# Pearbiossom-M/FlashAttention-from-Scratch-with-Triton

Hardware: AMD Instinct MI355X
Metric: achieved TFLOPS fwd and fwd+bwd (B=4,H=32,N=4096,D=64 causal); %MFMA peak (higher is better)
Workload: dtype bf16

## Files before the change

### flashattention-from-scratch-with-triton_amd/csrc/fa_fwd_v4.hip

```cpp
#include <stdlib.h>

#include <type_traits>

#include "fa_common.h"
#include "fa_kernels.h"

namespace fa {

template <int D_>
struct Fwd4Cfg {
  static constexpr int D = D_;
  static constexpr int BM = 256, NT = 256, NW = 4;
  static constexpr int BN = D == 64 ? 128 : 64;
  static constexpr int NBUF = D == 64 ? 3 : 4;
  static constexpr int NKB = BN / 32;
  static constexpr int ROWB = D * 2, CPR = D / 8, KS = D / 16, DB = D / 32;
  static constexpr int TILE_BYTES = BN * ROWB;
  static constexpr int V_BASE = NBUF * TILE_BYTES;
  static constexpr int FLAG_OFF = 2 * NBUF * TILE_BYTES;
  static constexpr int RB_BYTES = 32 * ROWB;
  static constexpr int QS_OFF = FLAG_OFF + 16;
  static constexpr int QS_BYTES = D == 64 ? 8 * RB_BYTES : 0;
  static constexpr int LDS_BYTES = QS_OFF + QS_BYTES;
  static constexpr int PIECES = TILE_BYTES / (NW * 1024);
  static constexpr int RPI = 1024 / ROWB;
#ifndef FA_FWD4_LSUM_MFMA
#define FA_FWD4_LSUM_MFMA 0
#endif
  static constexpr bool LSUM = FA_FWD4_LSUM_MFMA && D == 64;
  static constexpr int PVG = 2 * DB + (LSUM ? 2 : 0);
  static constexpr int NSS = 2 * KS, NPV = 2 * PVG, NSLOT = NSS + NPV;
  static constexpr int INFLIGHT = (NBUF - 3) * 2 * PIECES;
};

template <typename T> struct Fwd4Limit;
template <> struct Fwd4Limit<BF16> { static constexpr float value = 1.2676506e30f; };
template <> struct Fwd4Limit<FP16> { static constexpr float value = 32768.0f; };

#ifdef FA_STAMPS
#define FA4_STAMP(slot)                                                           \
  do {                                                                            \
    __builtin_amdgcn_sched_barrier(0);                                            \
    unsigned long long now_;                                                      \
    asm volatile("s_memtime %0\n\ts_waitcnt lgkmcnt(0)" : "=s"(now_)::"memory"); \
    __builtin_amdgcn_sched_barrier(0);                                            \
    seg[slot] += now_ - last_;                                                    \
    last_ = now_;                                                                 \
  } while (0)
#else
#define FA4_STAMP(slot) do {} while (0)
#endif

template <int D, typename T, bool CAUSAL>
__global__ __launch_bounds__(256, 1) void fa_fwd4_kernel(FwdParams p) {
#ifdef FA_STAMPS
  unsigned long long clk0_, rt0_;
  asm volatile("s_memtime %0\n\ts_memrealtime %1\n\ts_waitcnt lgkmcnt(0)" : "=s"(clk0_), "=s"(rt0_)::"memory");
  unsigned long long seg[12] = {0, 0, 0, 0, 0, 0, 0, 0, 0, 0, 0, 0};
  unsigned long long last_ = clk0_, ntile_ = 0, npass_ = 0;
#endif
  using C = Fwd4Cfg<D>;
  using vec8 = typename T::vec8;
  constexpr bool FOLD = T::kFoldScale;
  constexpr bool CHAIN_M = FOLD;
  extern __shared__ __attribute__((aligned(16))) char smem_raw[];
  FA_LDS char* smem = (FA_LDS char*)smem_raw;

  const int tid = threadIdx.x;
  const int lane = tid & 63;
  const int wave = __builtin_amdgcn_readfirstlane(tid >> 6);
  const int r = lane & 31, h = lane >> 5;

  const bool CONT = CAUSAL || (p.Sk % C::BN == 0 && p.Sk / C::BN >= C::NBUF - 1);
  constexpr bool STAGEQ = D == 64;
  const bool paired = CAUSAL && p.pair;
  const int nq = p.nq_tiles;
  const int per_bh = paired ? (nq + 1) / 2 : nq;
  const int n_items = per_bh * p.B * p.H;
  const int Sq = p.Sq, Sk = p.Sk;
  struct Work {
    int b, h, idx, npass;
  };
  auto decode = [&](int item) __attribute__((always_inline)) -> Work {
    const int w = xcd_remap(item, n_items);
    const int bh = p.div_per_bh.div(w), idx = w - bh * per_bh, b = p.div_h.div(bh);
    return Work{b, bh - b * p.H, idx, (paired && idx != nq - 1 - idx) ? 2 : 1};
  };
  auto tile_of = [&](const Work& wk, int pass) __attribute__((always_inline)) -> int {
    return paired ? (pass == 0 ? nq - 1 - wk.idx : wk.idx) : (CAUSAL ? nq - 1 - wk.idx : wk.idx);
  };

  const int q_rs = p.lq.rs, kv_rs = p.lk.rs, o_rs = p.lo.rs;
  auto rsrc_q = [&](const Work& wk, bool valid) __attribute__((always_inline)) {
    return make_rsrc((const char*)p.q + wk.b * p.lq.sb + wk.h * p.lq.sh, valid ? view_bytes(Sq, q_rs, C::ROWB) : 0u);
  };
  auto rsrc_k = [&](const Work& wk, bool valid) __attribute__((always_inline)) {
    return make_rsrc((const char*)p.k + wk.b * p.lk.sb + wk.h * p.lk.sh, valid ? view_bytes(Sk, kv_rs, C::ROWB) : 0u);
  };
  auto rsrc_v = [&](const Work& wk, bool valid) __attribute__((always_inline)) {
    return make_rsrc((const char*)p.v + wk.b * p.lv.sb + wk.h * p.lv.sh, valid ? view_bytes(Sk, kv_rs, C::ROWB) : 0u);
  };

  int dma_src[C::PIECES];
#pragma unroll
  for (int i = 0; i < C::PIECES; ++i) {
    const int row = (C::BN / C::NW) * wave + C::RPI * i + lane / C::CPR;
    dma_src[i] = row * kv_rs + swz_chunk<D>(row, lane % C::CPR) * 16 - 1024 * (i & 1);
  }
  int k_off[C::KS];
#pragma unroll
  for (int ks = 0; ks < C::KS; ++ks) k_off[ks] = lds_off<D>(r, 2 * ks + h);
  int v_off[2][C::DB];
#pragma unroll
  for (int e = 0; e < 2; ++e)
#pragma unroll
    for (int db = 0; db < C::DB; ++db) v_off[e][db] = tr_lane_off<D>(lane, 8 * e, db);
  const float c2 = p.scale * kLog2e;

  if (Sk % C::BN != 0) {
    lds_zero_fill(smem, C::FLAG_OFF, C::NT, tid);
    __syncthreads();
  }

  if (tid == 0) *(FA_LDS int*)(smem + C::FLAG_OFF) = 0;
  bool primed = false;
  int r0 = 0;

  int item = blockIdx.x, pass = 0;
  Work wk = decode(item);
  Work nwk_item = decode(min(item + (int)gridDim.x, n_items - 1));
  for (;;) {
    const int b_ = wk.b, h_ = wk.h;
    const __amdgpu_buffer_rsrc_t rk = rsrc_k(wk, true), rv = rsrc_v(wk, true);
    const __amdgpu_buffer_rsrc_t ro = make_rsrc((char*)p.o + b_ * p.lo.sb + h_ * p.lo.sh, view_bytes(Sq, o_rs, C::ROWB));
    const __amdgpu_buffer_rsrc_t rl = make_rsrc(p.lse + b_ * p.lse_sb + h_ * p.lse_sh, (unsigned)Sq * 4);
    const bool more_pass = pass + 1 < wk.npass, more_item = item + (int)gridDim.x < n_items;
    const bool has_next = CONT && (more_pass || more_item);
    const Work nwk = more_pass ? wk : nwk_item;
    const int nq0_wg = tile_of(nwk, more_pass ? pass + 1 : 0) * C::BM;

    FA4_STAMP(8);
    const int q0_wg = tile_of(wk, pass) * C::BM;
    const int qw = q0_wg + 32 * wave;
    auto qrow = [&](int rb) __attribute__((always_inline)) { return qw + 128 * rb; };

    const int kv_end = CAUSAL ? min(Sk, q0_wg + C::BM) : Sk;
    const int ntiles = (kv_end + C::BN - 1) / C::BN;
    const int nplain = CAUSAL ? min(Sk / C::BN, q0_wg / C::BN) : Sk / C::BN;

    auto dma_pair_of = [&](const __amdgpu_buffer_rsrc_t& rkx, const __amdgpu_buffer_rsrc_t& rvx, int t, int slot, int j) __attribute__((always_inline)) {
      constexpr int HALF = C::PIECES / 2;
      const int i = 2 * (j % HALF);
      const int dst = slot * C::TILE_BYTES + ((C::BN / C::NW) * wave + C::RPI * i) * C::ROWB;
      if (j < HALF) dma_pieces<2>(rkx, lds_addr_of(smem + dst), dma_src + i, t * C::BN * kv_rs);
      else dma_pieces<2>(rvx, lds_addr_of(smem + C::V_BASE + dst), dma_src + i, t * C::BN * kv_rs);
    };
    auto dma_pair = [&](int t, int slot, int j) __attribute__((always_inline)) { dma_pair_of(rk, rv, t, slot, j); };
    auto fetch_tile = [&](int t, int slot) __attribute__((always_inline)) {
#pragma unroll
      for (int j = 0; j < C::PIECES; ++j) dma_pair(t, slot, j);
    };
    auto stage_q_pair = [&](const __amdgpu_buffer_rsrc_t& rqx, int q0, int rb, int hf) __attribute__((always_inline)) {
      if constexpr (STAGEQ) {
        const int prow = lane >> 3;
        int voff[2];
#pragma unroll
        for (int i = 0; i < 2; ++i) {
          const int row = 8 * (2 * hf + i) + prow;
          voff[i] = (q0 + 128 * rb + 32 * wave + row) * q_rs + swz_chunk<D>(row, lane & 7) * 16 - 1024 * i;
        }
        dma_pieces<2>(rqx, lds_addr_of(smem + C::QS_OFF + (2 * wave + rb) * C::RB_BYTES + 2048 * hf), voff, 0);
      }
    };
    const bool was_primed = primed;
    if (!primed) {
      r0 = 0;
      if constexpr (STAGEQ) {
        const __amdgpu_buffer_rsrc_t rq = rsrc_q(wk, true);
#pragma unroll
        for (int g = 0; g < 4; ++g) stage_q_pair(rq, q0_wg, g >> 1, g & 1);
      }
#pragma unroll
      for (int t = 0; t < C::NBUF - 1; ++t) fetch_tile(t, t);
    }
    FA4_STAMP(9);
    u32x4 qf[2][C::KS];
    if constexpr (STAGEQ) {
      if (!was_primed) __builtin_amdgcn_s_waitcnt(0x0F70 | (((C::NBUF - 1) * 2 * C::PIECES) & 15) | ((((C::NBUF - 1) * 2 * C::PIECES) >> 4) << 14));
      asm volatile("" ::: "memory");
#pragma unroll
      for (int rb = 0; rb < 2; ++rb)
#pragma unroll
        for (int ks = 0; ks < C::KS; ++ks) {
          vec8 q = as_vec8<T>(lds_read16(smem + C::QS_OFF + (2 * wave + rb) * C::RB_BYTES + k_off[ks]));
          if constexpr (FOLD) q = scale_frag<T>(q, c2);
          qf[rb][ks] = __builtin_bit_cast(u32x4, q);
        }
    } else {
      const __amdgpu_buffer_rsrc_t rq = rsrc_q(wk, true);
#pragma unroll
      for (int rb = 0; rb < 2; ++rb)
#pragma unroll
        for (int ks = 0; ks < C::KS; ++ks) {
          vec8 q = as_vec8<T>(buf_load16(rq, (qrow(rb) + r) * q_rs + (2 * ks + h) * 16));
          if constexpr (FOLD) q = scale_frag<T>(q, c2);
          qf[rb][ks] = __builtin_bit_cast(u32x4, q);
        }
    }
    FA4_STAMP(10);
    int mask_base[2];
#pragma unroll
    for (int rb = 0; rb < 2; ++rb) mask_base[rb] = (CAUSAL ? min(qrow(rb) + r, Sk - 1) : Sk - 1) - 4 * h;

    auto commit = [&]() __attribute__((always_inline)) {
      asm volatile("" ::: "memory");
#ifdef FA_FWD4_COMMIT_LGKM0
      __builtin_amdgcn_s_waitcnt(0x0070 | (C::INFLIGHT & 15) | ((C::INFLIGHT >> 4) << 14));
#else
      __builtin_amdgcn_s_waitcnt(0x0F70 | (C::INFLIGHT & 15) | ((C::INFLIGHT >> 4) << 14));
#endif
      __builtin_amdgcn_s_barrier();
      asm volatile("" ::: "memory");
    };

    f32x16 S_[2][2];
    f32x16 negm[CHAIN_M ? 2 : 1];
    float mrow[2], nmc[2];
    float l[2];
    u32x4 pk[2][2][2];
#ifdef FA_FWD4_KR_FULL
    constexpr int KR = C::KS;
#else
    constexpr int KR = C::KS < 4 ? C::KS : 4;
#endif
    u32x4 KF[KR];
    vec8 VF[2 * C::DB];
    f32x16 oacc[2][C::DB];
    f32x16 lacc[C::LSUM ? 2 : 1];
    const unsigned one2 = std::is_same<T, BF16>::value ? 0x3F803F80u : 0x3C003C00u;
    const u32x4 ones = {one2, one2, one2, one2};
    int thr[2][2];

    auto block_valu = [&](int tau, f32x16 (&X)[2], u32x4 (&PK)[2][2], const int (&TH)[2], auto mask_tag, auto has0_tag) __attribute__((always_inline)) {
      constexpr bool MASK = decltype(mask_tag)::value, HAS0 = decltype(has0_tag)::value;
      auto first_q = [](int t) { return t <= 0 ? 0 : (32 * t + C::NSLOT - 1) / C::NSLOT; };
      auto work = [&](int t, bool exps) __attribute__((always_inline)) {
        if (t < 0 || t >= C::NSLOT) return;
#pragma unroll
        for (int u = 0; u < 2; ++u) {
          const int q = first_q(t) + u;
          if (q >= first_q(t + 1) || q >= 32) continue;
          const int rb = (q >> 3) & 1, e = (q & 7) + 8 * (q >> 4);
          if (rb == 0 && !HAS0) continue;
          if (exps) {
            float x = CHAIN_M ? X[rb][e] : (FOLD ? X[rb][e] + nmc[rb] : __builtin_fmaf(X[rb][e], c2, nmc[rb]));
            if constexpr (MASK) x = (e & 3) + 8 * (e >> 2) > TH[rb] ? -INFINITY : x;
            X[rb][e] = __builtin_amdgcn_exp2f(x);
          } else {
            if constexpr (!C::LSUM) l[rb] += X[rb][e];
            if (q & 1) {
              const int j = e >> 1;
              PK[rb][j >> 2][j & 3] = pack2<T>(X[rb][e - 1], X[rb][e]);
            }
          }
        }
      };
      work(tau - C::NSS, true);
      work(tau - 1 - C::NSS, false);
    };
    auto block_iter = [&](auto j_tag, auto set_tag, auto mode_tag, auto pst_tag, int kb0, const int (&kc)[C::KS], int kc_imm,
                          const int (&kn)[C::KS], int kn_delta, int kn_imm,
                          const int (&vc)[2][C::DB], int vc_imm, int vp0, int vp1, int vp_imm,
                          auto&& hook) __attribute__((always_inline)) {
      constexpr int J = decltype(j_tag)::value, SET = decltype(set_tag)::value, PSET = SET ^ 1;
      constexpr int MODE = decltype(mode_tag)::value, PST = decltype(pst_tag)::value;
      constexpr bool OWN0 = MODE != 3, PREV0 = PST != 2;
      using OwnMask = std::integral_constant<bool, MODE != 0>;
      using PrevMask = std::integral_constant<bool, PST != 0>;
      if constexpr (MODE != 0) {
        thr[SET][0] = mask_base[0] - kb0;
        thr[SET][1] = MODE == 2 ? (1 << 20) : mask_base[1] - kb0;
      }
#pragma unroll
      for (int s = 0; s < C::NSLOT; ++s) {
        hook(J, s);
        if (s < C::NSS) {
          const int ks = s >> 1, rb = s & 1;
          if (rb == 1 || OWN0) {
            if (ks == 0) {
              if constexpr (CHAIN_M) T::mfma_v_first(S_[SET][rb], KF[0], qf[rb][0], negm[CHAIN_M ? rb : 0]);
              else T::mfma_v_first0(S_[SET][rb], KF[0], qf[rb][0]);
            } else {
              T::mfma_v_acc(S_[SET][rb], KF[ks % KR], qf[rb][ks]);
            }
          }
        } else {
          const int n = s - C::NSS, e = n / C::PVG, m = n % C::PVG, rb = m & 1;
          if (rb == 1 || PREV0) {
            if (m < 2 * C::DB) oacc[rb][m >> 1] = T::mfma(VF[e * C::DB + (m >> 1)], as_vec8<T>(pk[PSET][rb][e]), oacc[rb][m >> 1]);
            else lacc[rb] = T::mfma(as_vec8<T>(ones), as_vec8<T>(pk[PSET][rb][e]), lacc[rb]);
          }
        }
        if (s >= 2 && s <= C::NSS && (s & 1) == 0) {
          const int ks = (s - 2) >> 1, nk = ks + KR;
          if (nk < C::KS) KF[ks % KR] = lds_read16(lds_at(kc[nk] + kc_imm));
          else KF[ks % KR] = lds_read16(lds_at(kn[nk - C::KS] + kn_delta + kn_imm));
        }
#pragma unroll
        for (int pp = 0; pp < 2 * C::DB; ++pp) {
          const int e = pp / C::DB, db = pp % C::DB, at = C::NSS + e * C::PVG + 2 * db + 2;
          if (at < C::NSLOT && s == at)
            VF[pp] = lds_read_tr_frag<T>(lds_at(vc[0][db] + vc_imm + 16 * e * C::ROWB), lds_at(vc[1][db] + vc_imm + 16 * e * C::ROWB));
          if (at >= C::NSLOT && s == 0)
            VF[pp] = lds_read_tr_frag<T>(lds_at(vp0 + vp_imm), lds_at(vp1 + vp_imm));
        }
        block_valu(C::NSLOT + s, S_[PSET], pk[PSET], thr[PSET], PrevMask{}, std::integral_constant<bool, PREV0>{});
        block_valu(s, S_[SET], pk[SET], thr[SET], OwnMask{}, std::integral_constant<bool, OWN0>{});
        if constexpr (CHAIN_M) {
          if (s == 1 && OWN0) keep_live(negm[0]);
          if (s == 2) keep_live(negm[CHAIN_M ? 1 : 0]);
        }
        __builtin_amdgcn_sched_barrier(0);
      }
    };
    auto drain = [&](auto set_tag, auto pst_tag, int rt_last) __attribute__((always_inline)) {
      constexpr int PSET = decltype(set_tag)::value ^ 1, PST = decltype(pst_tag)::value;
      constexpr bool PREV0 = PST != 2;
      if constexpr (!C::LSUM) {
        const int base = C::V_BASE + rt_last * C::TILE_BYTES + (C::NKB - 1) * 32 * C::ROWB + 16 * C::ROWB;
        VF[2 * C::DB - 1] = lds_read_tr_frag<T>(smem + v_off[0][C::DB - 1] + base, smem + v_off[1][C::DB - 1] + base);
      }
#pragma unroll
      for (int s = 0; s < C::NSLOT; ++s) {
        if (s >= C::NSS) {
          const int n = s - C::NSS, e = n / C::PVG, m = n % C::PVG, rb = m & 1;
          if (rb == 1 || PREV0) {
            if (m < 2 * C::DB) oacc[rb][m >> 1] = T::mfma(VF[e * C::DB + (m >> 1)], as_vec8<T>(pk[PSET][rb][e]), oacc[rb][m >> 1]);
            else lacc[rb] = T::mfma(as_vec8<T>(ones), as_vec8<T>(pk[PSET][rb][e]), lacc[rb]);
          }
        }
        block_valu(C::NSLOT + s, S_[PSET], pk[PSET], thr[PSET], std::integral_constant<bool, PST != 0>{}, std::integral_constant<bool, PREV0>{});
        __builtin_amdgcn_sched_barrier(0);
      }
    };

    auto tile_step = [&](int t, int rt, auto mode_tag, auto pst_tag, auto nx_tag) __attribute__((always_inline)) {
      constexpr int MODE = decltype(mode_tag)::value, NX = decltype(nx_tag)::value;
      const __amdgpu_buffer_rsrc_t nrk = rsrc_k(nwk, has_next && NX != 0), nrv = rsrc_v(nwk, has_next && NX != 0);
      const __amdgpu_buffer_rsrc_t nrq = rsrc_q(nwk, has_next && NX == 2);
      using OwnSt = std::integral_constant<int, MODE == 0 ? 0 : (MODE == 3 ? 2 : 1)>;
      const int rn = rt + 1 == C::NBUF ? 0 : rt + 1, rp = rt == 0 ? C::NBUF - 1 : rt - 1;
      const int lds0 = (int)lds_addr_of(smem);
      int kA[C::KS], vA[2][C::DB], vP[2];
      const int kdelta = (rn - rt) * C::TILE_BYTES;
#pragma unroll
      for (int ks = 0; ks < C::KS; ++ks) {
        kA[ks] = opaque(lds0 + k_off[ks] + rt * C::TILE_BYTES);
      }
#pragma unroll
      for (int e = 0; e < 2; ++e) {
#pragma unroll
        for (int db = 0; db < C::DB; ++db) vA[e][db] = opaque(lds0 + v_off[e][db] + C::V_BASE + rt * C::TILE_BYTES);
        vP[e] = opaque(lds0 + v_off[e][C::DB - 1] + C::V_BASE + (t == 0 ? rt * C::TILE_BYTES
                                                                  : rp * C::TILE_BYTES + (C::NKB - 1) * 32 * C::ROWB) + 16 * C::ROWB);
      }
      auto hook = [&](int J, int s) __attribute__((always_inline)) {
        if (J == C::NKB - 1) {
          if (s == 1) commit();
#pragma unroll
          for (int j = 0; j < C::PIECES; ++j)
            if (s == C::NSS + 1 + 2 * j) {
              if constexpr (NX != 0) dma_pair_of(nrk, nrv, t + C::NBUF - 1 - ntiles, rp, j);
              else dma_pair(t + C::NBUF - 1, rp, j);
            }
        }
        if constexpr (NX == 2 && STAGEQ) {
          if (J < 2 && s == C::NSS + 1) stage_q_pair(nrq, nq0_wg, J, 0);
          if (J < 2 && s == C::NSS + 5) stage_q_pair(nrq, nq0_wg, J, 1);
        }
      };
      auto go = [&](auto j_tag) __attribute__((always_inline)) {
        constexpr int J = decltype(j_tag)::value;
        constexpr int kPrevImm = (J - 1) * 32 * C::ROWB + 16 * C::ROWB;
        if constexpr (J == 0)
          block_iter(j_tag, std::integral_constant<int, 0>{}, mode_tag, pst_tag, t * C::BN, kA, 0, kA, 0, 32 * C::ROWB, vA, 0, vP[0], vP[1], 0, hook);
        else if constexpr (J + 1 < C::NKB)
          block_iter(j_tag, std::integral_constant<int, J & 1>{}, mode_tag, OwnSt{}, t * C::BN + 32 * J, kA, J * 32 * C::ROWB, kA, 0,
                     (J + 1) * 32 * C::ROWB, vA, J * 32 * C::ROWB, vA[0][C::DB - 1], vA[1][C::DB - 1], kPrevImm, hook);
        else
          block_iter(j_tag, std::integral_constant<int, J & 1>{}, mode_tag, OwnSt{}, t * C::BN + 32 * J, kA, J * 32 * C::ROWB, kA, kdelta, 0,
                     vA, J * 32 * C::ROWB, vA[0][C::DB - 1], vA[1][C::DB - 1], kPrevImm, hook);
      };
      go(std::integral_constant<int, 0>{});
      go(std::integral_constant<int, 1>{});
      if constexpr (C::NKB == 4) {
        go(std::integral_constant<int, 2>{});
        go(std::integral_constant<int, 3>{});
      }
    };

    auto scout_block = [&](const FA_LDS char* kblk, int kb0, float (&mx)[2]) __attribute__((always_inline)) {
#pragma unroll
      for (int rb = 0; rb < 2; ++rb) {
        f32x16 s;
        T::mfma_v_first0(s, lds_read16(kblk + k_off[0]), qf[rb][0]);
#pragma unroll
        for (int ks = 1; ks < C::KS; ++ks) T::mfma_v_acc(s, lds_read16(kblk + k_off[ks]), qf[rb][ks]);
        settle_mfma(s);
        const int th = opaque(mask_base[rb] - kb0);
        float mm = mx[rb];
#pragma unroll
        for (int i = 0; i < 16; ++i) mm = __builtin_fmaxf(mm, (i & 3) + 8 * (i >> 2) > th ? -INFINITY : s[i]);
        mx[rb] = mm;
      }
    };
    auto set_m = [&](const float (&mx)[2]) __attribute__((always_inline)) {
#pragma unroll
      for (int rb = 0; rb < 2; ++rb) {
        const float m = half_max(mx[rb]);
        mrow[rb] = m > -INFINITY ? m : 0.f;
        nmc[rb] = FOLD ? -mrow[rb] : -mrow[rb] * c2;
        if constexpr (CHAIN_M) {
#pragma unroll
          for (int i = 0; i < 16; ++i) negm[rb][i] = -mrow[rb];
        }
      }
    };

    for (int attempt = 0; attempt < 2; ++attempt) {
      if (attempt == 1) {
        r0 = 0;
#pragma unroll
        for (int t = 0; t < C::NBUF - 1; ++t) fetch_tile(t, t);
      }
      if (!was_primed || attempt == 1) {
        asm volatile("" ::: "memory");
        __builtin_amdgcn_s_waitcnt(0x0070 | (((C::NBUF - 2) * 2 * C::PIECES) & 15) | ((((C::NBUF - 2) * 2 * C::PIECES) >> 4) << 14));
        __builtin_amdgcn_s_barrier();
        asm volatile("" ::: "memory");
      }

      FA4_STAMP(0);
      float mx[2] = {-INFINITY, -INFINITY};
      if (attempt == 0) {
        scout_block(smem + r0 * C::TILE_BYTES, 0, mx);
        set_m(mx);
      } else {
        for (int t = 0; t < ntiles; ++t) {
          if (t > 0) {
            __syncthreads();
            fetch_tile(t, t % C::NBUF);
            __builtin_amdgcn_s_waitcnt(0x0070);
            __syncthreads();
          }
          for (int j = 0; j < C::NKB; ++j)
            scout_block(smem + (t % C::NBUF) * C::TILE_BYTES + j * 32 * C::ROWB, t * C::BN + 32 * j, mx);
        }
        set_m(mx);
        __builtin_amdgcn_s_waitcnt(0x0070);
        __syncthreads();
#pragma unroll
        for (int t = 0; t < C::NBUF - 1; ++t) fetch_tile(t, t);
        asm volatile("" ::: "memory");
        __builtin_amdgcn_s_waitcnt(0x0070 | (((C::NBUF - 2) * 2 * C::PIECES) & 15) | ((((C::NBUF - 2) * 2 * C::PIECES) >> 4) << 14));
        __builtin_amdgcn_s_barrier();
        asm volatile("" ::: "memory");
      }

      FA4_STAMP(1);
#pragma unroll
      for (int rb = 0; rb < 2; ++rb) {
        l[rb] = 0.f;
#pragma unroll
        for (int i = 0; i < 16; ++i) {
          const int q = (i >> 3) * 16 + rb * 8 + (i & 7);
          S_[1][rb][i] = C::NSS + q * C::NSLOT / 32 < C::NSLOT ? 0.f : -INFINITY;
        }
#pragma unroll
        for (int e = 0; e < 2; ++e) pk[1][rb][e] = u32x4{0u, 0u, 0u, 0u};
#pragma unroll
        for (int db = 0; db < C::DB; ++db)
#pragma unroll
          for (int i = 0; i < 16; ++i) oacc[rb][db][i] = 0.f;
        if constexpr (C::LSUM) {
#pragma unroll
          for (int i = 0; i < 16; ++i) lacc[rb][i] = 0.f;
        }
        thr[0][rb] = thr[1][rb] = 1 << 20;
      }
#pragma unroll
      for (int ks = 0; ks < KR; ++ks) KF[ks] = lds_read16(smem + r0 * C::TILE_BYTES + k_off[ks]);
#pragma unroll
      for (int pp = 0; pp < 2 * C::DB; ++pp) VF[pp] = as_vec8<T>(u32x4{0u, 0u, 0u, 0u});
      __builtin_amdgcn_sched_barrier(0);

      FA4_STAMP(2);
      int t = 0, rt = r0;
      using I0 = std::integral_constant<int, 0>;
      using I1 = std::integral_constant<int, 1>;
      using I2 = std::integral_constant<int, 2>;
      using I3 = std::integral_constant<int, 3>;
      const int nloop = (!CAUSAL && CONT) ? nplain - (C::NBUF - 1) : nplain;
      for (; t < nloop; ++t, rt = rt + 1 == C::NBUF ? 0 : rt + 1) tile_step(t, rt, I0{}, I0{}, I0{});
#ifdef FA_STAMPS
      FA4_STAMP(3);
      ntile_ += nplain;
      ++npass_;
#endif
      constexpr int RT = 256 / C::BN;
      auto nxt = [](int x) __attribute__((always_inline)) { return x + 1 == C::NBUF ? 0 : x + 1; };
      if constexpr (CAUSAL) {
        int rt_last;
        if constexpr (RT == 2) {
          tile_step(t, rt, I2{}, I1{}, I2{});
          tile_step(t + 1, rt_last = nxt(rt), I3{}, I1{}, I1{});
        } else {
          tile_step(t, rt, I2{}, I1{}, I0{});
          tile_step(t + 1, nxt(rt), I2{}, I1{}, I1{});
          tile_step(t + 2, nxt(nxt(rt)), I3{}, I1{}, I1{});
          tile_step(t + 3, rt_last = nxt(nxt(nxt(rt))), I3{}, I2{}, I1{});
        }
        static_assert(C::NBUF - 1 == (RT == 2 ? 2 : 3), "the masked tiles carry exactly the next pass's first NBUF - 1 tiles");
        FA4_STAMP(4);
        drain(I0{}, I2{}, rt_last);
        rt = rt_last;
      } else {
        if (CONT) {
          if constexpr (C::NBUF == 3) {
            tile_step(t, rt, I0{}, I0{}, I2{});
            tile_step(t + 1, nxt(rt), I0{}, I0{}, I1{});
            rt = nxt(nxt(rt));
          } else {
            tile_step(t, rt, I0{}, I0{}, I1{});
            tile_step(t + 1, nxt(rt), I0{}, I0{}, I1{});
            tile_step(t + 2, nxt(nxt(rt)), I0{}, I0{}, I1{});
            rt = nxt(nxt(nxt(rt)));
          }
          t += C::NBUF - 1;
        }
        for (; t < ntiles; ++t, rt = nxt(rt)) tile_step(t, rt, I1{}, I1{}, I0{});
        rt = rt == 0 ? C::NBUF - 1 : rt - 1;
        FA4_STAMP(4);
        drain(I0{}, I1{}, rt);
      }
      FA4_STAMP(5);

      float lt[2];
      bool bad = false;
#pragma unroll
      for (int rb = 0; rb < 2; ++rb) {
        lt[rb] = C::LSUM ? lacc[C::LSUM ? rb : 0][0] : half_sum(l[rb]);
        bad = bad || !(lt[rb] <= Fwd4Limit<T>::value);
      }
      FA_LDS int* flag = (FA_LDS int*)(smem + C::FLAG_OFF);
      if (attempt == 0 && __builtin_amdgcn_ballot_w64(bad) != 0 && lane == 0) *flag = 1;
      if (CONT) __builtin_amdgcn_s_waitcnt(0x0070 | (((C::NBUF - 2) * 2 * C::PIECES) & 15) | ((((C::NBUF - 2) * 2 * C::PIECES) >> 4) << 14));
      else __builtin_amdgcn_s_waitcnt(0x0070);
      __syncthreads();
      const int redo = __builtin_amdgcn_readfirstlane(*flag);
      FA4_STAMP(6);
      if (!redo) {
        FA_LDS char* stage = smem + (wave >> 1) * C::V_BASE + rt * C::TILE_BYTES + (wave & 1) * 32 * C::ROWB;
#pragma unroll
        for (int rb = 0; rb < 2; ++rb) {
          const float inv = lt[rb] > 0.f ? 1.0f / lt[rb] : 0.f;
          store_tile_rows<D, T>(oacc[rb], inv, stage, ro, qrow(rb) * o_rs, lane, o_rs);
          if (h == 0)
            buf_store_f32(rl, (qrow(rb) + r) * 4, mrow[rb] * (FOLD ? kLn2 : p.scale) + __builtin_logf(lt[rb]));
        }
        FA4_STAMP(7);
        primed = has_next;
        r0 = rt + 1 == C::NBUF ? 0 : rt + 1;
        break;
      }
      __builtin_amdgcn_s_waitcnt(0x0F70);
      __syncthreads();
      if (tid == 0) {
        *flag = 0;
#ifndef FA_STAMPS
        if (p.dbg) atomicAdd((unsigned*)p.dbg, 1u);
#endif
      }
    }
    if (more_pass) {
      ++pass;
    } else {
      item += gridDim.x;
      if (item >= n_items) break;
      wk = nwk_item;
      nwk_item = decode(min(item + (int)gridDim.x, n_items - 1));
      pass = 0;
    }
  }
#ifdef FA_STAMPS
  if (p.dbg && lane == 0) {
    unsigned long long* d = (unsigned long long*)p.dbg + ((size_t)blockIdx.x * 4 + wave) * 16;
    for (int i = 0; i < 12; ++i) d[i] = seg[i];
    d[12] = npass_;
    d[13] = ntile_;
    unsigned long long clk1_, rt1_;
    asm volatile("s_memtime %0\n\ts_memrealtime %1\n\ts_waitcnt lgkmcnt(0)" : "=s"(clk1_), "=s"(rt1_)::"memory");
    d[14] = clk1_ - clk0_;
    d[15] = rt1_ - rt0_;
  }
#endif
}

template <int D, typename T, bool CAUSAL>
static hipError_t launch4(const FwdParams& p, hipStream_t s) {
  using C = Fwd4Cfg<D>;
  int grid = (CAUSAL && p.pair ? (p.nq_tiles + 1) / 2 : p.nq_tiles) * p.B * p.H;
  if (CAUSAL || (p.Sk % C::BN == 0 && p.Sk / C::BN >= C::NBUF - 1)) {
    static std::atomic<int> cus{0};
    int n = cus.load(std::memory_order_relaxed);
    if (n == 0) {
      int dev = 0;
      if (hipGetDevice(&dev) != hipSuccess || hipDeviceGetAttribute(&n, hipDeviceAttributeMultiprocessorCount, dev) != hipSuccess || n < 8) n = 256;
      n -= n % 8;
      cus.store(n, std::memory_order_relaxed);
    }
    if (grid > n) grid = n;
  }
  auto kern = fa_fwd4_kernel<D, T, CAUSAL>;
  static std::atomic<unsigned long long> opted_in{0};
  if (hipError_t e = opt_in_lds((const void*)kern, C::LDS_BYTES, opted_in)) return e;
  hipLaunchKernelGGL(kern, dim3(grid), dim3(C::NT), C::LDS_BYTES, s, p);
  return hipGetLastError();
}

hipError_t launch_fwd_v4(FwdParams p, int D, int dtype, int causal, hipStream_t s) {
  p.nq_tiles = (p.Sq + 255) / 256;
  p.pair = causal != 0;
  p.div_per_bh = make_fastdiv(p.pair ? (p.nq_tiles + 1) / 2 : p.nq_tiles);
  p.div_h = make_fastdiv(p.H);
#define FA_GO(DD, TT) (causal ? launch4<DD, TT, true>(p, s) : launch4<DD, TT, false>(p, s))
  if (D == 64) return dtype == 1 ? FA_GO(64, BF16) : FA_GO(64, FP16);
  if (D == 128) return dtype == 1 ? FA_GO(128, BF16) : FA_GO(128, FP16);
#undef FA_GO
  return hipErrorInvalidValue;
}

}
```

Measured before the change: 888.7.

## Add per-wave diagonal walk for causal D=64 masked tiles with reversed Q row blocks

```diff
diff --git a/flashattention-from-scratch-with-triton_amd/csrc/fa_fwd_v4.hip b/flashattention-from-scratch-with-triton_amd/csrc/fa_fwd_v4.hip
--- a/flashattention-from-scratch-with-triton_amd/csrc/fa_fwd_v4.hip
+++ b/flashattention-from-scratch-with-triton_amd/csrc/fa_fwd_v4.hip
@@ -33,6 +33,9 @@
   static constexpr int INFLIGHT = (NBUF - 3) * 2 * PIECES;
 };
 
+constexpr int wait_vm(int n) { return 0x0F70 | (n & 15) | ((n >> 4) << 14); }
+constexpr int wait_vm_lgkm0(int n) { return 0x0070 | (n & 15) | ((n >> 4) << 14); }
+
 template <typename T> struct Fwd4Limit;
 template <> struct Fwd4Limit<BF16> { static constexpr float value = 1.2676506e30f; };
 template <> struct Fwd4Limit<FP16> { static constexpr float value = 32768.0f; };
@@ -116,6 +119,8 @@
 #pragma unroll
     for (int db = 0; db < C::DB; ++db) v_off[e][db] = tr_lane_off<D>(lane, 8 * e, db);
   const float c2 = p.scale * kLog2e;
+  const int qblk1 = D == 64 ? 128 + 32 * (3 - wave) : 128 + 32 * wave;
+  auto qblk = [&](int rb) __attribute__((always_inline)) { return D == 64 && rb == 1 ? qblk1 : 32 * wave + 128 * rb; };
 
   if (Sk % C::BN != 0) {
     lds_zero_fill(smem, C::FLAG_OFF, C::NT, tid);
@@ -142,7 +147,7 @@
     FA4_STAMP(8);
     const int q0_wg = tile_of(wk, pass) * C::BM;
     const int qw = q0_wg + 32 * wave;
-    auto qrow = [&](int rb) __attribute__((always_inline)) { return qw + 128 * rb; };
+    auto qrow = [&](int rb) __attribute__((always_inline)) { return D == 64 && rb == 1 ? q0_wg + qblk1 : qw + 128 * rb; };
 
     const int kv_end = CAUSAL ? min(Sk, q0_wg + C::BM) : Sk;
     const int ntiles = (kv_end + C::BN - 1) / C::BN;
@@ -167,7 +172,7 @@
 #pragma unroll
         for (int i = 0; i < 2; ++i) {
           const int row = 8 * (2 * hf + i) + prow;
-          voff[i] = (q0 + 128 * rb + 32 * wave + row) * q_rs + swz_chunk<D>(row, lane & 7) * 16 - 1024 * i;
+          voff[i] = (q0 + qblk(rb) + row) * q_rs + swz_chunk<D>(row, lane & 7) * 16 - 1024 * i;
         }
         dma_pieces<2>(rqx, lds_addr_of(smem + C::QS_OFF + (2 * wave + rb) * C::RB_BYTES + 2048 * hf), voff, 0);
       }
@@ -274,10 +279,10 @@
                           auto&& hook) __attribute__((always_inline)) {
       constexpr int J = decltype(j_tag)::value, SET = decltype(set_tag)::value, PSET = SET ^ 1;
       constexpr int MODE = decltype(mode_tag)::value, PST = decltype(pst_tag)::value;
-      constexpr bool OWN0 = MODE != 3, PREV0 = PST != 2;
-      using OwnMask = std::integral_constant<bool, MODE != 0>;
-      using PrevMask = std::integral_constant<bool, PST != 0>;
-      if constexpr (MODE != 0) {
+      constexpr bool OWN0 = MODE < 3, PREV0 = PST < 2;
+      using OwnMask = std::integral_constant<bool, MODE >= 1 && MODE <= 3>;
+      using PrevMask = std::integral_constant<bool, PST == 1 || PST == 2>;
+      if constexpr (OwnMask::value) {
         thr[SET][0] = mask_base[0] - kb0;
         thr[SET][1] = MODE == 2 ? (1 << 20) : mask_base[1] - kb0;
       }
@@ -323,11 +328,11 @@
         __builtin_amdgcn_sched_barrier(0);
       }
     };
-    auto drain = [&](auto set_tag, auto pst_tag, int rt_last) __attribute__((always_inline)) {
+    auto drain = [&](auto set_tag, auto pst_tag, int rt_last, int kb_last = C::NKB - 1) __attribute__((always_inline)) {
       constexpr int PSET = decltype(set_tag)::value ^ 1, PST = decltype(pst_tag)::value;
-      constexpr bool PREV0 = PST != 2;
+      constexpr bool PREV0 = PST < 2;
       if constexpr (!C::LSUM) {
-        const int base = C::V_BASE + rt_last * C::TILE_BYTES + (C::NKB - 1) * 32 * C::ROWB + 16 * C::ROWB;
+        const int base = C::V_BASE + rt_last * C::TILE_BYTES + kb_last * 32 * C::ROWB + 16 * C::ROWB;
         VF[2 * C::DB - 1] = lds_read_tr_frag<T>(smem + v_off[0][C::DB - 1] + base, smem + v_off[1][C::DB - 1] + base);
       }
 #pragma unroll
@@ -339,7 +344,7 @@
             else lacc[rb] = T::mfma(as_vec8<T>(ones), as_vec8<T>(pk[PSET][rb][e]), lacc[rb]);
           }
         }
-        block_valu(C::NSLOT + s, S_[PSET], pk[PSET], thr[PSET], std::integral_constant<bool, PST != 0>{}, std::integral_constant<bool, PREV0>{});
+        block_valu(C::NSLOT + s, S_[PSET], pk[PSET], thr[PSET], std::integral_constant<bool, PST == 1 || PST == 2>{}, std::integral_constant<bool, PREV0>{});
         __builtin_amdgcn_sched_barrier(0);
       }
     };
@@ -348,7 +353,7 @@
       constexpr int MODE = decltype(mode_tag)::value, NX = decltype(nx_tag)::value;
       const __amdgpu_buffer_rsrc_t nrk = rsrc_k(nwk, has_next && NX != 0), nrv = rsrc_v(nwk, has_next && NX != 0);
       const __amdgpu_buffer_rsrc_t nrq = rsrc_q(nwk, has_next && NX == 2);
-      using OwnSt = std::integral_constant<int, MODE == 0 ? 0 : (MODE == 3 ? 2 : 1)>;
+      using OwnSt = std::integral_constant<int, MODE == 0 ? 0 : (MODE == 3 ? 2 : (MODE == 4 ? 3 : 1))>;
       const int rn = rt + 1 == C::NBUF ? 0 : rt + 1, rp = rt == 0 ? C::NBUF - 1 : rt - 1;
       const int lds0 = (int)lds_addr_of(smem);
       int kA[C::KS], vA[2][C::DB], vP[2];
@@ -427,6 +432,107 @@
       }
     };
 
+    constexpr bool WALK = CAUSAL && C::NBUF == 3 && STAGEQ;
+    constexpr int WALK_COMMIT_VM = 0;
+    constexpr int END_CHECK_VM = WALK ? 0 : (C::NBUF - 2) * 2 * C::PIECES;
+    static_assert(!WALK || (C::NKB == 4 && C::PIECES == 4 && C::KS == 4 && KR == C::KS),
+                  "the walk's visit plan, DMA slots and fragment reads assume D = 64: 128-key tiles of four 32-key blocks");
+    auto diag_walk = [&](int t, int ra) __attribute__((always_inline)) {
+      if constexpr (WALK) {
+        const int rbs = ra + 1 == C::NBUF ? 0 : ra + 1, rpv = ra == 0 ? C::NBUF - 1 : ra - 1;
+        const int lds0 = (int)lds_addr_of(smem);
+        const int kdelta = (rbs - ra) * C::TILE_BYTES;
+        auto go = [&](auto w_tag) __attribute__((always_inline)) {
+          constexpr int W = decltype(w_tag)::value;
+          constexpr int NIT = 8 - W;
+          constexpr int ICOMMIT = W == 0 ? 3 : 2;
+          int kA[C::KS], vA[2][C::DB], vP[2], kB[C::KS], vB[2][C::DB];
+#pragma unroll
+          for (int ks = 0; ks < C::KS; ++ks) kA[ks] = opaque(lds0 + k_off[ks] + ra * C::TILE_BYTES);
+#pragma unroll
+          for (int e = 0; e < 2; ++e) {
+#pragma unroll
+            for (int db = 0; db < C::DB; ++db) vA[e][db] = opaque(lds0 + v_off[e][db] + C::V_BASE + ra * C::TILE_BYTES);
+            vP[e] = opaque(lds0 + v_off[e][C::DB - 1] + C::V_BASE + (t == 0 ? ra * C::TILE_BYTES
+                                                                       : rpv * C::TILE_BYTES + (C::NKB - 1) * 32 * C::ROWB) + 16 * C::ROWB);
+          }
+          const __amdgpu_buffer_rsrc_t nrk = rsrc_k(nwk, has_next), nrv = rsrc_v(nwk, has_next);
+          const __amdgpu_buffer_rsrc_t nrq = rsrc_q(nwk, has_next);
+          auto hook = [&](int i, int s) __attribute__((always_inline)) {
+            if (i == ICOMMIT) {
+              if (s == 1) {
+                asm volatile("" ::: "memory");
+                __builtin_amdgcn_s_waitcnt(wait_vm(WALK_COMMIT_VM));
+                __builtin_amdgcn_s_barrier();
+                asm volatile("" ::: "memory");
+              }
+#pragma unroll
+              for (int j = 0; j < C::PIECES; ++j)
+                if (s == C::NSS + 1 + 2 * j) dma_pair_of(nrk, nrv, 0, rpv, j);
+            }
+            if (i == ICOMMIT + 1) {
+#pragma unroll
+              for (int g = 0; g < 4; ++g)
+                if (s == C::NSS + 1 + 2 * g) stage_q_pair(nrq, nq0_wg, g >> 1, g & 1);
+            }
+          };
+          static_assert(ICOMMIT + 1 < NIT, "every wave has an iteration after the commit for the Q rows");
+          auto it = [&](auto i_tag) __attribute__((always_inline)) {
+            constexpr int I = decltype(i_tag)::value;
+            constexpr bool TB = I >= 4;
+            constexpr int J = TB ? I - 4 : I;
+            auto mode_of = [](int x) { return x < 4 ? (x < W ? 0 : (x == W ? 2 : 4)) : (x - 4 < 3 - W ? 4 : 3); };
+            auto st_of = [](int m) { return m == 0 ? 0 : (m == 2 ? 1 : (m == 3 ? 2 : 3)); };
+            constexpr int MODE = mode_of(I), PST = I == 0 ? 0 : st_of(mode_of(I - 1));
+            using Mo = std::integral_constant<int, MODE>;
+            using Ps = std::integral_constant<int, PST>;
+            using Se = std::integral_constant<int, I & 1>;
+            const int kb0 = (t + (TB ? 1 : 0)) * C::BN + 32 * J;
+            auto h = [&](int, int s) __attribute__((always_inline)) { hook(I, s); };
+            const int(&kc)[C::KS] = TB ? kB : kA;
+            const int(&vc)[2][C::DB] = TB ? vB : vA;
+            if constexpr (I == 0)
+              block_iter(i_tag, Se{}, Mo{}, Ps{}, kb0, kc, 0, kc, 0, 32 * C::ROWB, vc, 0, vP[0], vP[1], 0, h);
+            else if constexpr (I == NIT - 1)
+              block_iter(i_tag, Se{}, Mo{}, Ps{}, kb0, kc, J * 32 * C::ROWB, kc, 0, J * 32 * C::ROWB, vc, J * 32 * C::ROWB,
+                         (J == 0 ? vA : vc)[0][C::DB - 1], (J == 0 ? vA : vc)[1][C::DB - 1],
+                         (J == 0 ? C::NKB - 1 : J - 1) * 32 * C::ROWB + 16 * C::ROWB, h);
+            else if constexpr (I == 3)
+              block_iter(i_tag, Se{}, Mo{}, Ps{}, kb0, kA, 3 * 32 * C::ROWB, kA, kdelta, 0, vA, 3 * 32 * C::ROWB,
+                         vA[0][C::DB - 1], vA[1][C::DB - 1], 2 * 32 * C::ROWB + 16 * C::ROWB, h);
+            else if constexpr (I == 4)
+              block_iter(i_tag, Se{}, Mo{}, Ps{}, kb0, kB, 0, kB, 0, 32 * C::ROWB, vB, 0,
+                         vA[0][C::DB - 1], vA[1][C::DB - 1], 3 * 32 * C::ROWB + 16 * C::ROWB, h);
+            else
+              block_iter(i_tag, Se{}, Mo{}, Ps{}, kb0, kc, J * 32 * C::ROWB, kc, 0, (J + 1) * 32 * C::ROWB, vc, J * 32 * C::ROWB,
+                         vc[0][C::DB - 1], vc[1][C::DB - 1], (J - 1) * 32 * C::ROWB + 16 * C::ROWB, h);
+          };
+          it(std::integral_constant<int, 0>{});
+          it(std::integral_constant<int, 1>{});
+          it(std::integral_constant<int, 2>{});
+          it(std::integral_constant<int, 3>{});
+#pragma unroll
+          for (int ks = 0; ks < C::KS; ++ks) kB[ks] = opaque(lds0 + k_off[ks] + rbs * C::TILE_BYTES);
+#pragma unroll
+          for (int e = 0; e < 2; ++e)
+#pragma unroll
+            for (int db = 0; db < C::DB; ++db) vB[e][db] = opaque(lds0 + v_off[e][db] + C::V_BASE + rbs * C::TILE_BYTES);
+          it(std::integral_constant<int, 4>{});
+          if constexpr (NIT > 5) it(std::integral_constant<int, 5>{});
+          if constexpr (NIT > 6) it(std::integral_constant<int, 6>{});
+          if constexpr (NIT > 7) it(std::integral_constant<int, 7>{});
+          FA4_STAMP(4);
+          drain(std::integral_constant<int, NIT & 1>{}, std::integral_constant<int, 2>{}, rbs, 3 - W);
+        };
+        switch (wave) {
+          case 0: go(std::integral_constant<int, 0>{}); break;
+          case 1: go(std::integral_constant<int, 1>{}); break;
+          case 2: go(std::integral_constant<int, 2>{}); break;
+          default: go(std::integral_constant<int, 3>{}); break;
+        }
+      }
+    };
+
     for (int attempt = 0; attempt < 2; ++attempt) {
       if (attempt == 1) {
         r0 = 0;
@@ -510,20 +616,21 @@
       constexpr int RT = 256 / C::BN;
       auto nxt = [](int x) __attribute__((always_inline)) { return x + 1 == C::NBUF ? 0 : x + 1; };
       if constexpr (CAUSAL) {
-        int rt_last;
-        if constexpr (RT == 2) {
-          tile_step(t, rt, I2{}, I1{}, I2{});
-          tile_step(t + 1, rt_last = nxt(rt), I3{}, I1{}, I1{});
+        static_assert(WALK == (RT == 2), "128-key tiles take the walk, 64-key tiles the lock-step masked tiles");
+        if constexpr (WALK) {
+          diag_walk(t, rt);
+          rt = nxt(rt);
         } else {
+          int rt_last;
           tile_step(t, rt, I2{}, I1{}, I0{});
           tile_step(t + 1, nxt(rt), I2{}, I1{}, I1{});
           tile_step(t + 2, nxt(nxt(rt)), I3{}, I1{}, I1{});
           tile_step(t + 3, rt_last = nxt(nxt(nxt(rt))), I3{}, I2{}, I1{});
-        }
-        static_assert(C::NBUF - 1 == (RT == 2 ? 2 : 3), "the masked tiles carry exactly the next pass's first NBUF - 1 tiles");
-        FA4_STAMP(4);
-        drain(I0{}, I2{}, rt_last);
-        rt = rt_last;
+          static_assert(WALK || C::NBUF - 1 == 3, "the masked tiles carry exactly the next pass's first NBUF - 1 tiles");
+          FA4_STAMP(4);
+          drain(I0{}, I2{}, rt_last);
+          rt = rt_last;
+        }
       } else {
         if (CONT) {
           if constexpr (C::NBUF == 3) {
@@ -554,12 +661,18 @@
       }
       FA_LDS int* flag = (FA_LDS int*)(smem + C::FLAG_OFF);
       if (attempt == 0 && __builtin_amdgcn_ballot_w64(bad) != 0 && lane == 0) *flag = 1;
-      if (CONT) __builtin_amdgcn_s_waitcnt(0x0070 | (((C::NBUF - 2) * 2 * C::PIECES) & 15) | ((((C::NBUF - 2) * 2 * C::PIECES) >> 4) << 14));
+      if (CONT) __builtin_amdgcn_s_waitcnt(wait_vm_lgkm0(END_CHECK_VM));
       else __builtin_amdgcn_s_waitcnt(0x0070);
       __syncthreads();
       const int redo = __builtin_amdgcn_readfirstlane(*flag);
       FA4_STAMP(6);
       if (!redo) {
+        if constexpr (WALK) {
+          const int ra = rt == 0 ? C::NBUF - 1 : rt - 1;
+          const __amdgpu_buffer_rsrc_t nrk = rsrc_k(nwk, has_next), nrv = rsrc_v(nwk, has_next);
+#pragma unroll
+          for (int j = 0; j < C::PIECES; ++j) dma_pair_of(nrk, nrv, 1, ra, j);
+        }
         FA_LDS char* stage = smem + (wave >> 1) * C::V_BASE + rt * C::TILE_BYTES + (wave & 1) * 32 * C::ROWB;
 #pragma unroll
         for (int rb = 0; rb < 2; ++rb) {
```

Measured after the change: 894.0, median of 6. About the same (+0.6%).
